# Biblbrox/ViT-Spectre-Experiments

Measured on AMD Instinct MI355X. Metric: images/sec training, Spectre-ViT-S CIFAR-100 bs512, higher is better.
Workload: dtype bf16; 1 GPU; Spectre-ViT-Small (E512 H16 F768 L4 P4 N65, 100 classes, dropout 0.001), fft mixer, train step fwd+CE+bwd+AdamW, bs 512/GPU; mixer=fft, global_batch=512, parallelism=dp1

## Files before the change

### vit-spectre-experiments_amd/csrc/spv_gemm.hip

```cpp
#define SPV_USES_SEED
#include "spv_common.h"
#include "spv_gemm_core.h"

#include <stdlib.h>

#include <algorithm>
#include <type_traits>

namespace {

constexpr int BM = GEMM_BM, BN = GEMM_BN;
constexpr int ROWB = 128 + 16;
constexpr int KBYTES = 128;

template <typename T> struct KT { static constexpr int BK = KBYTES / sizeof(T); static constexpr int CH = 16 / sizeof(T); };

template <typename TO> __device__ __forceinline__ void store_out(TO* p, float v);
template <> __device__ __forceinline__ void store_out<float>(float* p, float v) { *p = v; }
template <> __device__ __forceinline__ void store_out<bf16_t>(bf16_t* p, float v) { *p = f2bf(v); }
template <typename TO> __device__ __forceinline__ float load_out(const TO* p);
template <> __device__ __forceinline__ float load_out<float>(const float* p) { return *p; }
template <> __device__ __forceinline__ float load_out<bf16_t>(const bf16_t* p) { return bf2f(*p); }

__device__ __forceinline__ int xcd_remap(int id, int nwg) {
    int q = nwg >> 3, r = nwg & 7, x = id & 7;
    int base = (x < r) ? x * (q + 1) : r * (q + 1) + (x - r) * q;
    return base + (id >> 3);
}

__device__ __forceinline__ void tile_coords(int tile, int tiles_n, int tiles_mn, int& tm, int& tn) {
    constexpr int GM = 8;
    if (tiles_n <= 8) { tm = tile / tiles_n; tn = tile % tiles_n; return; }
    const int tiles_m = tiles_mn / tiles_n;
    const int per_group = GM * tiles_n;
    const int grp = tile / per_group, in = tile % per_group;
    const int m_first = grp * GM;
    const int gm = min(GM, tiles_m - m_first);
    tm = m_first + in % gm;
    tn = in / gm;
}

template <typename TO>
__device__ __forceinline__ void store_acc_tile(f32x16 (*acc)[2], unsigned char* smem, const float* __restrict__ bias,
                                               TO* __restrict__ C, float* __restrict__ ws, int M, int N, int ldc, int accumulate,
                                               int m0, int n0, int split, int rg, int gs, int roff,
                                               const float* __restrict__ bias2d, const void* __restrict__ bc = nullptr,
                                               int bc_pw = 0, int bc_bf = 0, int wrow = -1, int wcol = -1, float drop_p = 0.0f,
                                               uint64_t drop_seed = 0) {
    const int lane = threadIdx.x & 63, wave = threadIdx.x >> 6;
    const int fh = lane >> 5;
    if (wrow < 0) wrow = (wave >> 1) * 64;
    if (wcol < 0) wcol = (wave & 1) * 64;
    float* stage = reinterpret_cast<float*>(smem + wave * 9216);
    constexpr int SLD = 68;
    const bool vec_c = ((size_t)ldc * sizeof(TO)) % 16 == 0 && ((reinterpret_cast<uintptr_t>(C) | reinterpret_cast<uintptr_t>(bias)) & 15) == 0;
    const bool vec_ws = (N & 3) == 0;
    const uint64_t seed_live = drop_p > 0.0f ? live_seed(drop_seed) : 0;
#pragma unroll
    for (int i = 0; i < 2; ++i) {
        __syncthreads();
#pragma unroll
        for (int j = 0; j < 2; ++j)
#pragma unroll
            for (int r = 0; r < 16; ++r)
                stage[((r & 3) + 8 * (r >> 2) + 4 * fh) * SLD + j * 32 + (lane & 31)] = acc[i][j][r];
        __syncthreads();
#pragma unroll
        for (int t = 0; t < 4; ++t) {
            const int qd = lane + 64 * t;
            const int lr = qd >> 3, c8 = qd & 7;
            const int row = m0 + wrow + i * 32 + lr;
            const int col0 = n0 + wcol + c8 * 8;
            if (row >= M || col0 >= N) continue;
            float v[8];
            {
                const float4 lo = *reinterpret_cast<const float4*>(stage + lr * SLD + c8 * 8);
                const float4 hi = *reinterpret_cast<const float4*>(stage + lr * SLD + c8 * 8 + 4);
                v[0] = lo.x; v[1] = lo.y; v[2] = lo.z; v[3] = lo.w; v[4] = hi.x; v[5] = hi.y; v[6] = hi.z; v[7] = hi.w;
            }
            const int nvalid = min(8, N - col0);
            if (ws != nullptr) {
                float* wp = ws + ((size_t)split * M + row) * N + col0;
                if (nvalid == 8 && vec_ws) {
                    *reinterpret_cast<float4*>(wp) = make_float4(v[0], v[1], v[2], v[3]);
                    *reinterpret_cast<float4*>(wp + 4) = make_float4(v[4], v[5], v[6], v[7]);
                } else {
                    for (int u = 0; u < nvalid; ++u) wp[u] = v[u];
                }
                continue;
            }
            int orow = row;
            const float* b2 = nullptr;
            if (rg > 0) {
                orow = (row / rg) * gs + roff + (row % rg);
                if (bias2d) b2 = bias2d + (size_t)(row % rg) * N + col0;
            }
            TO* cp = C + (size_t)orow * ldc + col0;
            if (bc != nullptr) {
                const float sc = 1.0f / (float)bc_pw;
                const int ldp = N / bc_pw;
                if ((bc_pw & 7) == 0) {
                    const size_t o = (size_t)row * ldp + col0 / bc_pw;
                    const float t = (bc_bf ? bf2f(static_cast<const bf16_t*>(bc)[o]) : static_cast<const float*>(bc)[o]) * sc;
#pragma unroll
                    for (int u = 0; u < 8; ++u) v[u] += t;
                } else {
#pragma unroll
                    for (int u = 0; u < 8; ++u) {
                        if (u < nvalid) {
                            const size_t o = (size_t)row * ldp + (col0 + u) / bc_pw;
                            v[u] += (bc_bf ? bf2f(static_cast<const bf16_t*>(bc)[o]) : static_cast<const float*>(bc)[o]) * sc;
                        }
                    }
                }
            }
            if (nvalid == 8 && vec_c) {
                if (bias != nullptr) {
                    const float4 b0 = *reinterpret_cast<const float4*>(bias + col0), b1 = *reinterpret_cast<const float4*>(bias + col0 + 4);
                    v[0] += b0.x; v[1] += b0.y; v[2] += b0.z; v[3] += b0.w; v[4] += b1.x; v[5] += b1.y; v[6] += b1.z; v[7] += b1.w;
                }
                if (b2 != nullptr) {
                    if (vec_ws && (reinterpret_cast<uintptr_t>(bias2d) & 15) == 0) {
                        const float4 p0 = *reinterpret_cast<const float4*>(b2), p1 = *reinterpret_cast<const float4*>(b2 + 4);
                        v[0] += p0.x; v[1] += p0.y; v[2] += p0.z; v[3] += p0.w; v[4] += p1.x; v[5] += p1.y; v[6] += p1.z; v[7] += p1.w;
                    } else {
#pragma unroll
                        for (int u = 0; u < 8; ++u) v[u] += b2[u];
                    }
                }
                if (drop_p > 0.0f) {
                    const size_t fi = (size_t)orow * ldc + col0;
                    const unsigned key = dropout_row_key(seed_live, (uint64_t)fi >> 12);
                    const unsigned c0 = (unsigned)(fi & 4095);
                    const float inv_keep = 1.0f / (1.0f - drop_p);
                    const unsigned key_next = c0 > 4088u ? dropout_row_key(seed_live, ((uint64_t)fi >> 12) + 1) : key;
#pragma unroll
                    for (int u = 0; u < 8; ++u) v[u] *= dropout_scale(c0 + u < 4096u ? key : key_next, (c0 + u) & 4095u, drop_p, inv_keep);
                }
                if constexpr (sizeof(TO) == 2) {
                    if (accumulate) {
                        const uint4 old = *reinterpret_cast<const uint4*>(cp);
                        v[0] += __uint_as_float(old.x << 16); v[1] += __uint_as_float(old.x & 0xffff0000u);
                        v[2] += __uint_as_float(old.y << 16); v[3] += __uint_as_float(old.y & 0xffff0000u);
                        v[4] += __uint_as_float(old.z << 16); v[5] += __uint_as_float(old.z & 0xffff0000u);
                        v[6] += __uint_as_float(old.w << 16); v[7] += __uint_as_float(old.w & 0xffff0000u);
                    }
                    uint4 o;
                    o.x = pack_bf16x2(v[0], v[1]);
                    o.y = pack_bf16x2(v[2], v[3]);
                    o.z = pack_bf16x2(v[4], v[5]);
                    o.w = pack_bf16x2(v[6], v[7]);
                    *reinterpret_cast<uint4*>(cp) = o;
                } else {
                    float4* c4 = reinterpret_cast<float4*>(cp);
                    if (accumulate) {
                        const float4 o0 = c4[0], o1 = c4[1];
                        v[0] += o0.x; v[1] += o0.y; v[2] += o0.z; v[3] += o0.w; v[4] += o1.x; v[5] += o1.y; v[6] += o1.z; v[7] += o1.w;
                    }
                    c4[0] = make_float4(v[0], v[1], v[2], v[3]);
                    c4[1] = make_float4(v[4], v[5], v[6], v[7]);
                }
            } else {
                for (int u = 0; u < nvalid; ++u) {
                    float x = v[u];
                    if (bias != nullptr) x += bias[col0 + u];
                    if (b2 != nullptr) x += b2[u];
                    if (drop_p > 0.0f) {
                        const size_t fi = (size_t)orow * ldc + col0 + u;
                        x *= dropout_scale(dropout_row_key(seed_live, (uint64_t)fi >> 12), (unsigned)(fi & 4095), drop_p, 1.0f / (1.0f - drop_p));
                    }
                    if (accumulate) x += load_out<TO>(cp + u);
                    store_out<TO>(cp + u, x);
                }
            }
        }
    }
}

template <typename T, typename TO>
__global__ __launch_bounds__(256) void gemm_nt_kernel(const T* __restrict__ A, const T* __restrict__ B,
                                                      const float* __restrict__ bias, TO* __restrict__ C,
                                                      float* __restrict__ ws, int M, int N, int K, int lda,
                                                      int ldb, int ldc, int k_per_split, int accumulate,
                                                      int tiles_n, int tiles_mn, int nsplit, int rg, int gs, int roff,
                                                      const float* __restrict__ bias2d, const void* __restrict__ bc, int bc_pw,
                                                      int bc_bf, float drop_p, uint64_t drop_seed) {
    constexpr int BK = KT<T>::BK;
    constexpr int CH = KT<T>::CH;
    __shared__ __attribute__((aligned(16))) unsigned char smem[2 * BM * ROWB];
    unsigned char* sA = smem;
    unsigned char* sB = smem + BM * ROWB;

    const int tid = threadIdx.x;
    const int lane = tid & 63;
    const int wave = tid >> 6;
    const int wm = wave >> 1, wn = wave & 1;

    const int lin = xcd_remap(blockIdx.x, tiles_mn * nsplit);
    const int split = lin / tiles_mn;
    const int tile = lin % tiles_mn;
    int tm, tn;
    tile_coords(tile, tiles_n, tiles_mn, tm, tn);
// ... 901 lines not shown
            if (left == 3) step_noload(t + 1, a2, b2);
        }
        multiply(((nfull - 1) & 1) * WBUF, no{}, 0, a0, b0);
        __syncthreads();
    }
    if (krem > 0) {
        load_partial(kbeg + nfull * TBK, a0, b0);
        store_part(0, a0, b0, -1);
        __syncthreads();
        multiply(0, no{}, 0, a0, b0);
        __syncthreads();
    }
    store_acc_tile<TO>(acc, tw_smem, nullptr, C, ws, M, N, ldc, accumulate, m0, n0, split, 0, 0, 0, nullptr, nullptr, 0, 0, wm * 64, wn * 64);
}

constexpr int TW_SMEM_DB = 2 * (TBK * TWROWA + TBK * TROWB);
template <typename TO>
__global__ __launch_bounds__(512) void gemm_tn_wide_kernel(const bf16_t* __restrict__ A, const bf16_t* __restrict__ B, TO* __restrict__ C,
                                                           float* __restrict__ ws, int M, int N, int K, int lda, int ldb, int ldc,
                                                           int k_per_split, int accumulate, int tiles_n, int tiles_mn, int nsplit) {
    const int lin = xcd_remap(blockIdx.x, tiles_mn * nsplit);
    tn_wide_body<TO>(A, B, C, ws, M, N, K, lda, ldb, ldc, k_per_split, accumulate, tiles_n, lin % tiles_mn, lin / tiles_mn);
}

constexpr int TTM = GEMM_TTM;
constexpr int TTK = GEMM_TTK;
constexpr int TTROWA = TTM * 2 + 64;
constexpr int TT_SMEM = 2 * (TTK * TTROWA + TTK * TROWB);
template <typename TO>
__global__ __launch_bounds__(512) void gemm_tn_tall_kernel(const bf16_t* __restrict__ A, const bf16_t* __restrict__ B, TO* __restrict__ C,
                                                           float* __restrict__ ws, int M, int N, int K, int lda, int ldb, int ldc,
                                                           int k_per_split, int accumulate, int tiles_n, int tiles_mn, int nsplit) {
    extern __shared__ __attribute__((aligned(16))) unsigned char tt_smem[];
    constexpr int WBUF = TTK * TTROWA + TTK * TROWB;
    unsigned char* sA = tt_smem;
    unsigned char* sB = tt_smem + TTK * TTROWA;
    const int lin = xcd_remap(blockIdx.x, tiles_mn * nsplit);
    const int tile = lin % tiles_mn, split = lin / tiles_mn;
    const int tid = threadIdx.x, lane = tid & 63, wave = tid >> 6;
    const int wm = wave >> 1, wn = wave & 1;
    const int m0 = (tile / tiles_n) * TTM, n0 = (tile % tiles_n) * BN;
    const int kbeg = split * k_per_split;
    const int kend = min(K, kbeg + k_per_split);
    const int arow = tid >> 6, ach = tid & 63, brow = tid >> 4, bch = tid & 15;
    typedef tn_u32x4 RegA[4];
    RegA a0, a1, a2;
    tn_u32x4 b0, b1, b2;
    uint32_t aoff[4];
#pragma unroll
    for (int i = 0; i < 4; ++i) aoff[i] = (uint32_t)(((size_t)(arow + 8 * i) * lda + ach * 8) * 2);
    const uint32_t boff = (uint32_t)(((size_t)brow * ldb + bch * 8) * 2);
    const int nfull = (kend - kbeg) / TTK, krem = (kend - kbeg) % TTK;
    auto load_full = [&](int t, RegA& ra, tn_u32x4& rb) __attribute__((always_inline)) {
        const int k0 = kbeg + min(t, nfull - 1) * TTK;
        const unsigned char* ab = reinterpret_cast<const unsigned char*>(A + (size_t)k0 * lda + m0);
        const unsigned char* bb = reinterpret_cast<const unsigned char*>(B + (size_t)k0 * ldb + n0);
#pragma unroll
        for (int i = 0; i < 4; ++i) ra[i] = *reinterpret_cast<const tn_u32x4*>(ab + aoff[i]);
        rb = *reinterpret_cast<const tn_u32x4*>(bb + boff);
    };
    auto load_partial = [&](int k0, RegA& ra, tn_u32x4& rb) __attribute__((always_inline)) {
#pragma unroll
        for (int i = 0; i < 4; ++i) {
            const int k = k0 + arow + 8 * i;
            ra[i] = k < kend ? *reinterpret_cast<const tn_u32x4*>(A + (size_t)k * lda + m0 + ach * 8) : tn_u32x4{0u, 0u, 0u, 0u};
        }
        const int k = k0 + brow;
        rb = k < kend ? *reinterpret_cast<const tn_u32x4*>(B + (size_t)k * ldb + n0 + bch * 8) : tn_u32x4{0u, 0u, 0u, 0u};
    };
    auto store_part = [&](int buf, const RegA& ra, const tn_u32x4& rb, int ks) __attribute__((always_inline)) {
#pragma unroll
        for (int i = 0; i < 4; ++i)
            if (ks < 0 || ks == (i >= 3 ? 1 : 0)) *reinterpret_cast<tn_u32x4*>(sA + buf + (arow + 8 * i) * TTROWA + ach * 16) = ra[i];
        if (ks < 0 || ks == 1) *reinterpret_cast<tn_u32x4*>(sB + buf + brow * TROWB + bch * 16) = rb;
    };
    f32x16 acc[4][2];
#pragma unroll
    for (int i = 0; i < 4; ++i)
#pragma unroll
        for (int j = 0; j < 2; ++j)
#pragma unroll
            for (int r = 0; r < 16; ++r) acc[i][j][r] = 0.0f;
    const int g = lane >> 4, li = lane & 15, q = li >> 2, pp = li & 3;
    const unsigned char* fa0 = sA + (8 * (g >> 1) + q) * TTROWA + (16 * (g & 1) + 4 * pp) * 2 + (wm * 128) * 2;
    const unsigned char* fb0 = sB + (8 * (g >> 1) + q) * TROWB + (16 * (g & 1) + 4 * pp) * 2 + (wn * 64) * 2;
    using lds_ptr = s16x4 __attribute__((address_space(3)))*;
    auto fragA = [&](const unsigned char* p) __attribute__((always_inline)) {
        const s16x4 lo = __builtin_amdgcn_ds_read_tr16_b64_v4i16((lds_ptr)(p));
        const s16x4 hi = __builtin_amdgcn_ds_read_tr16_b64_v4i16((lds_ptr)(p + 4 * TTROWA));
        typedef __attribute__((ext_vector_type(8))) short s16x8;
        const s16x8 v = {lo[0], lo[1], lo[2], lo[3], hi[0], hi[1], hi[2], hi[3]};
        return __builtin_bit_cast(bf16x8, v);
    };
    auto multiply = [&](int cur, auto store_tag, int nxt, const RegA& ra, const tn_u32x4& rb) __attribute__((always_inline)) {
        constexpr bool STORE = decltype(store_tag)::value;
#pragma unroll
        for (int ks = 0; ks < TTK / 16; ++ks) {
            bf16x8 a[4], b[2];
#pragma unroll
            for (int f = 0; f < 4; ++f) a[f] = fragA(fa0 + cur + ks * 16 * TTROWA + f * 64);
#pragma unroll
            for (int f = 0; f < 2; ++f) b[f] = tr_frag(fb0 + cur + ks * 16 * TROWB + f * 64);
            if constexpr (STORE) store_part(nxt, ra, rb, ks);
#pragma unroll
            for (int i = 0; i < 4; ++i)
#pragma unroll
                for (int j = 0; j < 2; ++j)
                    acc[i][j] = __builtin_amdgcn_mfma_f32_32x32x16_bf16(a[i], b[j], acc[i][j], 0, 0, 0);
        }
    };
    using yes = std::true_type;
    using no = std::false_type;
    if (nfull > 0) {
        load_full(0, a0, b0);
        load_full(1, a1, b1);
        load_full(2, a2, b2);
        store_part(0, a0, b0, -1);
        load_full(3, a0, b0);
        __syncthreads();
        auto step = [&](int t, RegA& ra, tn_u32x4& rb) __attribute__((always_inline)) {
            multiply((t & 1) * WBUF, yes{}, ((t + 1) & 1) * WBUF, ra, rb);
            load_full(t + 4, ra, rb);
            __syncthreads();
        };
        auto step_noload = [&](int t, const RegA& ra, const tn_u32x4& rb) __attribute__((always_inline)) {
            multiply((t & 1) * WBUF, yes{}, ((t + 1) & 1) * WBUF, ra, rb);
            __syncthreads();
        };
        int t = 0;
        for (; t + 4 <= nfull; t += 3) {
            step(t, a1, b1);
            step(t + 1, a2, b2);
            step(t + 2, a0, b0);
        }
        const int left = nfull - t;
        if (left >= 2) {
            step_noload(t, a1, b1);
            if (left == 3) step_noload(t + 1, a2, b2);
        }
        multiply(((nfull - 1) & 1) * WBUF, no{}, 0, a0, b0);
        __syncthreads();
    }
    if (krem > 0) {
        load_partial(kbeg + nfull * TTK, a0, b0);
        store_part(0, a0, b0, -1);
        __syncthreads();
        multiply(0, no{}, 0, a0, b0);
        __syncthreads();
    }
    store_acc_tile<TO>(&acc[0], tt_smem, nullptr, C, ws, M, N, ldc, accumulate, m0, n0, split, 0, 0, 0, nullptr, nullptr, 0, 0, wm * 128, wn * 64);
    store_acc_tile<TO>(&acc[2], tt_smem, nullptr, C, ws, M, N, ldc, accumulate, m0, n0, split, 0, 0, 0, nullptr, nullptr, 0, 0, wm * 128 + 64, wn * 64);
}

__global__ __launch_bounds__(512) void gemm_tn_batch_wide_kernel(TnBatch tb, float* __restrict__ ws, int K, int k_per_split, int nsplit) {
    const TnWork w = tn_batch_work(tb, ws, K, k_per_split, nsplit);
    if (w.j < 0) return;
    const TnBatch::P& q = tb.p[w.j];
    tn_wide_body<float>(q.A, q.B, q.C, w.ws, q.M, q.N, w.K, q.lda, q.ldb, q.ldc, w.k_per_split, 0, q.tiles_n, w.tile, w.split);
}

template <typename TO>
__device__ __forceinline__ void splitk_reduce_body(const float* __restrict__ ws, const float* __restrict__ bias, TO* __restrict__ C, int M, int N,
                                                   int ldc, int splits, int accumulate, size_t bid, size_t nblocks, int tid, int nthreads) {
    const size_t total = (size_t)M * N;
    if ((N & 3) == 0) {
        const size_t quads = total >> 2;
        for (size_t qd = bid * nthreads + tid; qd < quads; qd += nblocks * nthreads) {
            const size_t e = qd << 2;
            const int row = (int)(e / N), col = (int)(e % N);
            float4 v = make_float4(0.0f, 0.0f, 0.0f, 0.0f);
            int sidx = 0;
            for (; sidx + 4 <= splits; sidx += 4) {
                const float4 a0 = *reinterpret_cast<const float4*>(ws + (size_t)(sidx + 0) * total + e);
                const float4 a1 = *reinterpret_cast<const float4*>(ws + (size_t)(sidx + 1) * total + e);
                const float4 a2 = *reinterpret_cast<const float4*>(ws + (size_t)(sidx + 2) * total + e);
                const float4 a3 = *reinterpret_cast<const float4*>(ws + (size_t)(sidx + 3) * total + e);
                v.x = (((v.x + a0.x) + a1.x) + a2.x) + a3.x;
                v.y = (((v.y + a0.y) + a1.y) + a2.y) + a3.y;
                v.z = (((v.z + a0.z) + a1.z) + a2.z) + a3.z;
                v.w = (((v.w + a0.w) + a1.w) + a2.w) + a3.w;
            }
            for (; sidx < splits; ++sidx) {
                const float4 a0 = *reinterpret_cast<const float4*>(ws + (size_t)sidx * total + e);
                v.x += a0.x; v.y += a0.y; v.z += a0.z; v.w += a0.w;
            }
            float o[4] = {v.x, v.y, v.z, v.w};
            TO* cp = C + (size_t)row * ldc + col;
#pragma unroll
            for (int u = 0; u < 4; ++u) {
                if (bias) o[u] += bias[col + u];
                if (accumulate) o[u] += load_out<TO>(cp + u);
                store_out<TO>(cp + u, o[u]);
            }
        }
        return;
    }
    for (size_t e = bid * nthreads + tid; e < total; e += nblocks * nthreads) {
        const int row = (int)(e / N), col = (int)(e % N);
        float v = 0.0f;
        for (int s = 0; s < splits; ++s) v += ws[(size_t)s * total + e];
        if (bias) v += bias[col];
        TO* cp = C + (size_t)row * ldc + col;
        if (accumulate) v += load_out<TO>(cp);
        store_out<TO>(cp, v);
    }
}

template <typename TO>
__global__ __launch_bounds__(256) void splitk_reduce_kernel(const float* __restrict__ ws, const float* __restrict__ bias,
                                                            TO* __restrict__ C, int M, int N, int ldc, int splits,
                                                            int accumulate) {
    splitk_reduce_body<TO>(ws, bias, C, M, N, ldc, splits, accumulate, blockIdx.x, gridDim.x, threadIdx.x, 256);
}

constexpr int FJ_MAX = GEMM_FJ_MAX;
static_assert(GEMM_FOLD_THREADS == FOLD_COLS * FOLD_ROWS, "spv_gemm_core.h sizes the batched reduce by the fold workgroup");
struct FoldJobs {
    int njobs;
    int first_block[FJ_MAX + 1];
    FoldJob job[FJ_MAX];
};
__device__ __forceinline__ void fold_jobs_block(const FoldJobs& fj, int bid, int tid) {
    int j = 0;
    while (j + 1 < fj.njobs && bid >= fj.first_block[j + 1]) ++j;
    fold_partials_block(fj.job[j], bid - fj.first_block[j], tid);
}
constexpr int FOLD_NARROW = 4;
__global__ __launch_bounds__(FOLD_COLS * FOLD_ROWS / FOLD_NARROW) void fold_multi_kernel(FoldJobs fj) {
    int j = 0;
    while (j + 1 < fj.njobs && (int)blockIdx.x >= fj.first_block[j + 1]) ++j;
    fold_partials_block<FOLD_NARROW>(fj.job[j], blockIdx.x - fj.first_block[j], threadIdx.x);
}

template <typename TO>
__global__ __launch_bounds__(FOLD_COLS * FOLD_ROWS) void splitk_reduce_fold_kernel(const float* __restrict__ ws, TO* __restrict__ C, int M, int N,
                                                                                   int ldc, int splits, int accumulate, int reduce_blocks,
                                                                                   FoldJobs fj) {
    const int fold_blocks = fj.first_block[fj.njobs];
    if ((int)blockIdx.x < fold_blocks)
        fold_jobs_block(fj, (int)blockIdx.x, threadIdx.x);
    else if (threadIdx.x < 256)
        splitk_reduce_body<TO>(ws, nullptr, C, M, N, ldc, splits, accumulate, blockIdx.x - fold_blocks, reduce_blocks, threadIdx.x, 256);
}

__global__ __launch_bounds__(FOLD_COLS * FOLD_ROWS) void splitk_reduce_batch_kernel(TnBatch tb, const float* __restrict__ ws, int splits,
                                                                                    int reduce_blocks, FoldJobs fj) {
    const int fold_blocks = fj.njobs > 0 ? fj.first_block[fj.njobs] : 0;
    if ((int)blockIdx.x < fold_blocks) {
        fold_jobs_block(fj, (int)blockIdx.x, threadIdx.x);
    } else {
        const int b = (int)blockIdx.x - fold_blocks;
        const int j = b / reduce_blocks;
        const TnBatch::P& q = tb.p[j];
        splitk_reduce_body<float>(ws + tb.ws_off[j], nullptr, q.C, q.M, q.N, q.ldc, splits, 0, b % reduce_blocks, reduce_blocks, threadIdx.x,
                                  FOLD_COLS * FOLD_ROWS);
    }
}

static thread_local float t_drop_p = 0.0f;
static thread_local uint64_t t_drop_seed = 0;

inline int ptr_lo(const void* p) { return p == nullptr ? -1 : (int)(reinterpret_cast<uintptr_t>(p) & 15); }

template <typename T, typename TO>
int launch_gemm(const GemmNtPlan& pl, const void* A, const void* B, const float* bias, void* C, int M, int N, int K, int lda, int ldb,
                int ldc, int accumulate, void* workspace, hipStream_t st, int rg, int gs, int roff, const float* bias2d, const void* bc,
                int bc_pw, int bc_bf) {
    const int tiles_m = cdiv(M, BM), tiles_n = cdiv(N, BN);
    const int splits = pl.splits, k_per_split = pl.k_per_split;
    float* ws = splits > 1 ? static_cast<float*>(workspace) : nullptr;
    const dim3 grid(pl.grid);
    switch (pl.kernel) {
    case GEMM_NT_ROWS:
        if constexpr (sizeof(T) == 2) {
            hipLaunchKernelGGL((gemm_nt_rows_kernel<TO>), grid, dim3(256), 0, st, static_cast<const bf16_t*>(A), static_cast<const bf16_t*>(B), bias,
                               static_cast<TO*>(C), M, N, K, lda, ldb, ldc, accumulate, cdiv(N, 32));
            SPV_LAUNCH_CHECK("spv_gemm_nt(rows)");
            SPV_COUNT_PATH(SPV_PATH_GEMM_ROWS);
            return 0;
        }
        return spv_set_error("spv_gemm_nt: the rows kernel takes bf16 operands");
    case GEMM_NT_STRIP:
        if constexpr (sizeof(T) == 2 && sizeof(TO) == 2) {
            const int nwg = pl.grid;
#define SPV_STRIP(MBV, EPIV)                                                                                                \
    hipLaunchKernelGGL((gemm_nt_strip_kernel<MBV, EPIV>), dim3(nwg), dim3(512), 0, st, static_cast<const bf16_t*>(A),       \
                       static_cast<const bf16_t*>(B), bias, static_cast<bf16_t*>(C), M, K, lda, ldb, ldc, pl.nstrips, pl.base, pl.rem, nwg, \
                       static_cast<const bf16_t*>(bc), bc_pw, bc ? N / bc_pw : 0)
#define SPV_STRIP_MB(EPIV)                  \
    do {                                    \
        if (pl.mb == 4) SPV_STRIP(4, EPIV); \
        else if (pl.mb == 3) SPV_STRIP(3, EPIV); \
        else SPV_STRIP(2, EPIV);            \
    } while (0)
            SPV_COUNT_PATH(pl.epi >= 2 ? SPV_PATH_GEMM_STRIP_POOL : pl.epi == 1 ? SPV_PATH_GEMM_STRIP_ACC : SPV_PATH_GEMM_STRIP);
            switch (pl.epi) {
            case 3: SPV_STRIP_MB(3); break;
            case 2: SPV_STRIP_MB(2); break;
            case 1: SPV_STRIP_MB(1); break;
            default: SPV_STRIP_MB(0); break;
            }
#undef SPV_STRIP_MB
#undef SPV_STRIP
            SPV_LAUNCH_CHECK("spv_gemm_nt(strip)");
            return 0;
        }
        return spv_set_error("spv_gemm_nt: the strip kernel takes bf16 operands and a bf16 output");
    case GEMM_NT_GLDS:
        if constexpr (sizeof(T) == 2) {
            hipLaunchKernelGGL((gemm_nt_glds_kernel<TO, 128, 2>), grid, dim3(256), 0, st, static_cast<const bf16_t*>(A),
                               static_cast<const bf16_t*>(B), bias, static_cast<TO*>(C), ws, M, N, K, lda, ldb, ldc, k_per_split,
// ... 124 lines not shown
static int gemm_tn_impl(const void* A, const void* B, void* C, int M, int N, int K, int lda, int ldb, int ldc, int out_dtype,
                        int accumulate, int splits, void* workspace, void* stream, const spv_fold_job* folds, int nfolds) {
    FoldJobs fj{};
    const int fold_blocks = fold_blocks_of(folds, nfolds, fj);
    const GemmTnPlan pl = gemm_tn_plan(out_dtype, M, N, K, lda, ldb, ldc, ptr_lo(A), ptr_lo(B), splits, ptr_lo(workspace), fold_blocks);
    SPV_CHECK(pl.kernel != GEMM_TN_REFUSE_EMPTY, "spv_gemm_tn: empty problem M=%d N=%d K=%d", M, N, K);
    SPV_CHECK(pl.kernel != GEMM_TN_REFUSE_DTYPE, "spv_gemm_tn: bad out_dtype %d", out_dtype);
    SPV_CHECK(pl.kernel != GEMM_TN_REFUSE_CHUNK, "spv_gemm_tn: M=%d N=%d lda=%d ldb=%d must be multiples of 8 (bf16, 16-byte chunks)", M, N, lda, ldb);
    SPV_CHECK(pl.kernel != GEMM_TN_REFUSE_ALIGN, "spv_gemm_tn: A/B must be 16-byte aligned");
    SPV_CHECK(pl.kernel != GEMM_TN_REFUSE_LD, "spv_gemm_tn: leading dimension too small");
    SPV_CHECK(pl.kernel != GEMM_TN_REFUSE_WORKSPACE, "spv_gemm_tn: split-K needs a 16-byte aligned workspace (splits=%d)", splits);
    SPV_CHECK(pl.kernel != GEMM_TN_REFUSE_FOLDS, "spv_gemm_tn_fold: 0..%d fold jobs, each with partials, parts > 0, nsum 1..5, n > 0 and out[0]", FJ_MAX);
    SPV_COUNT_PATH(SPV_PATH_GEMM_TN);
    hipStream_t st = static_cast<hipStream_t>(stream);
    const int tiles_m = cdiv(M, BM), tiles_n = cdiv(N, BN);
    splits = pl.splits;
    const int k_per_split = pl.k_per_split;
    float* ws = splits > 1 ? static_cast<float*>(workspace) : nullptr;
    const dim3 grid(pl.grid);
    const bool bf = out_dtype == SPV_BF16;
    switch (pl.kernel) {
    case GEMM_TN_TALL:
        if (bf) {
            (void)hipFuncSetAttribute(reinterpret_cast<const void*>(&gemm_tn_tall_kernel<bf16_t>), hipFuncAttributeMaxDynamicSharedMemorySize, TT_SMEM);
            hipLaunchKernelGGL((gemm_tn_tall_kernel<bf16_t>), grid, dim3(512), TT_SMEM, st, (const bf16_t*)A, (const bf16_t*)B, (bf16_t*)C, ws, M, N, K, lda, ldb,
                               ldc, k_per_split, accumulate, tiles_n, tiles_n, splits);
        } else {
            (void)hipFuncSetAttribute(reinterpret_cast<const void*>(&gemm_tn_tall_kernel<float>), hipFuncAttributeMaxDynamicSharedMemorySize, TT_SMEM);
            hipLaunchKernelGGL((gemm_tn_tall_kernel<float>), grid, dim3(512), TT_SMEM, st, (const bf16_t*)A, (const bf16_t*)B, (float*)C, ws, M, N, K, lda, ldb,
                               ldc, k_per_split, accumulate, tiles_n, tiles_n, splits);
        }
        SPV_LAUNCH_CHECK("spv_gemm_tn(tall)");
        break;
    case GEMM_TN_WIDE: {
        const int wt = (M / TWM) * tiles_n;
#define SPV_TNW(TOV)                                                                                                                      \
    do {                                                                                                                                  \
        (void)hipFuncSetAttribute(reinterpret_cast<const void*>(&gemm_tn_wide_kernel<TOV>), hipFuncAttributeMaxDynamicSharedMemorySize, TW_SMEM_DB); \
        hipLaunchKernelGGL((gemm_tn_wide_kernel<TOV>), grid, dim3(512), TW_SMEM_DB, st, (const bf16_t*)A, (const bf16_t*)B, (TOV*)C,     \
                           ws, M, N, K, lda, ldb, ldc, k_per_split, accumulate, tiles_n, wt, splits);                                     \
    } while (0)
        if (bf) SPV_TNW(bf16_t);
        else SPV_TNW(float);
#undef SPV_TNW
        SPV_LAUNCH_CHECK("spv_gemm_tn(wide)");
        SPV_COUNT_PATH(SPV_PATH_GEMM_TN_WIDE);
        break;
    }
    case GEMM_TN_TILE1:
    case GEMM_TN_TILE3:
#define SPV_TN(TOV, DV)                                                                                                     \
    hipLaunchKernelGGL((gemm_tn_kernel<TOV, DV>), grid, dim3(256), 0, st, (const bf16_t*)A, (const bf16_t*)B, (TOV*)C, ws, M, N, K, \
                       lda, ldb, ldc, k_per_split, accumulate, tiles_n, tiles_m * tiles_n, splits)
        if (bf) {
            if (pl.kernel == GEMM_TN_TILE1) SPV_TN(bf16_t, 1); else SPV_TN(bf16_t, 3);
        } else {
            if (pl.kernel == GEMM_TN_TILE1) SPV_TN(float, 1); else SPV_TN(float, 3);
        }
#undef SPV_TN
        SPV_LAUNCH_CHECK("spv_gemm_tn");
        break;
    default:
        return spv_set_error("spv_gemm_tn: no kernel for plan %d", (int)pl.kernel);
    }
    switch (pl.reduce) {
    case GEMM_TN_REDUCE_FOLDS:
        if (bf)
            hipLaunchKernelGGL((splitk_reduce_fold_kernel<bf16_t>), dim3(pl.reduce_blocks + fold_blocks), dim3(FOLD_COLS * FOLD_ROWS), 0, st, ws, (bf16_t*)C, M, N,
                               ldc, splits, accumulate, pl.reduce_blocks, fj);
        else
            hipLaunchKernelGGL((splitk_reduce_fold_kernel<float>), dim3(pl.reduce_blocks + fold_blocks), dim3(FOLD_COLS * FOLD_ROWS), 0, st, ws, (float*)C, M, N,
                               ldc, splits, accumulate, pl.reduce_blocks, fj);
        SPV_LAUNCH_CHECK("spv_gemm_tn_fold(split-k reduce + fold)");
        break;
    case GEMM_TN_REDUCE_PLAIN:
        if (bf)
            hipLaunchKernelGGL((splitk_reduce_kernel<bf16_t>), dim3(pl.reduce_blocks), dim3(256), 0, st, ws, (const float*)nullptr, (bf16_t*)C, M, N,
                               ldc, splits, accumulate);
        else
            hipLaunchKernelGGL((splitk_reduce_kernel<float>), dim3(pl.reduce_blocks), dim3(256), 0, st, ws, (const float*)nullptr, (float*)C, M, N, ldc,
                               splits, accumulate);
        SPV_LAUNCH_CHECK("spv_gemm_tn(split-k reduce)");
        break;
    case GEMM_TN_FOLD_ALONE:
        hipLaunchKernelGGL(fold_multi_kernel, dim3(fold_blocks), dim3(FOLD_COLS * FOLD_ROWS / FOLD_NARROW), 0, st, fj);
        SPV_LAUNCH_CHECK("spv_gemm_tn_fold(fold)");
        break;
    case GEMM_TN_NO_REDUCE:
        break;
    }
    return 0;
}

extern "C" int spv_gemm_tn(const void* A, const void* B, void* C, int M, int N, int K, int lda, int ldb, int ldc, int out_dtype,
                           int accumulate, int splits, void* workspace, void* stream) {
    return gemm_tn_impl(A, B, C, M, N, K, lda, ldb, ldc, out_dtype, accumulate, splits, workspace, stream, nullptr, 0);
}

extern "C" int spv_gemm_tn_fold(const void* A, const void* B, void* C, int M, int N, int K, int lda, int ldb, int ldc, int out_dtype,
                                int accumulate, int splits, void* workspace, const spv_fold_job* folds, int nfolds, void* stream) {
    return gemm_tn_impl(A, B, C, M, N, K, lda, ldb, ldc, out_dtype, accumulate, splits, workspace, stream, folds, nfolds);
}

extern "C" int spv_fold_multi(const spv_fold_job* folds, int nfolds, void* stream) {
    SPV_CHECK(folds != nullptr && nfolds > 0, "spv_fold_multi: no jobs");
    hipStream_t st = static_cast<hipStream_t>(stream);
    for (int j0 = 0; j0 < nfolds; j0 += FJ_MAX) {
        FoldJobs fj{};
        int blocks = 0;
        SPV_CHECK(fill_fold_jobs(folds + j0, std::min(FJ_MAX, nfolds - j0), fj, blocks) == 0, "spv_fold_multi: bad fold job");
        hipLaunchKernelGGL(fold_multi_kernel, dim3(blocks), dim3(FOLD_COLS * FOLD_ROWS / FOLD_NARROW), 0, st, fj);
        SPV_LAUNCH_CHECK("spv_fold_multi");
    }
    return 0;
}

static int gemm_tn_batch_impl(const spv_tn_problem* probs, int nprob, int K, int splits, void* workspace, const spv_fold_job* folds,
                              int nfolds, void* stream, int parts) {
    FoldJobs fj{};
    const int fold_blocks = fold_blocks_of(folds, nfolds, fj);
    GemmTnBatchProblem qs[TNB_MAX];
    const bool listed = probs != nullptr && nprob >= 1 && nprob <= TNB_MAX;
    for (int i = 0; listed && i < nprob; ++i) {
        const spv_tn_problem& q = probs[i];
        qs[i] = {q.m, q.n, q.lda, q.ldb, q.ldc, q.k, ptr_lo(q.a), ptr_lo(q.b), q.a != nullptr && q.b != nullptr && q.c != nullptr};
    }
    const GemmTnBatchPlan pl = gemm_tn_batch_plan(listed ? qs : nullptr, nprob, K, splits, ptr_lo(workspace), fold_blocks);
    SPV_CHECK(pl.kernel != GEMM_TNB_REFUSE_COUNT, "spv_gemm_tn_batch: 1..%d problems", TNB_MAX);
    SPV_CHECK(pl.kernel != GEMM_TNB_REFUSE_CALL, "spv_gemm_tn_batch: K=%d splits=%d need a 16-byte aligned workspace", K, splits);
    SPV_CHECK(pl.kernel != GEMM_TNB_REFUSE_FOLDS, "spv_gemm_tn_batch: 0..%d fold jobs, each with partials, parts > 0, nsum 1..5, n > 0 and out[0]", FJ_MAX);
    SPV_CHECK(pl.kernel != GEMM_TNB_REFUSE_K, "spv_gemm_tn_batch: problem %d: k must be 0 (= K) or 1..K=%d", pl.bad, K);
    SPV_CHECK(pl.kernel != GEMM_TNB_REFUSE_NO_LONG, "spv_gemm_tn_batch: no problem reduces over the call's K=%d rows", K);
    SPV_CHECK(pl.kernel != GEMM_TNB_REFUSE_EMPTY, "spv_gemm_tn_batch: empty problem %d", pl.bad);
    SPV_CHECK(pl.kernel != GEMM_TNB_REFUSE_SHAPE, "spv_gemm_tn_batch: problem %d: M, N, lda, ldb must be multiples of 8, leading dimensions >= extents", pl.bad);
    SPV_CHECK(pl.kernel != GEMM_TNB_REFUSE_ALIGN, "spv_gemm_tn_batch: problem %d: A/B must be 16-byte aligned", pl.bad);
    SPV_CHECK(pl.kernel != GEMM_TNB_REFUSE_SHORT_LDC, "spv_gemm_tn_batch: problem %d (short): ldc must be a multiple of 4", pl.bad);
    TnBatch tb{};
    tb.nprob = nprob;
    tb.nlong = pl.nlong;
    const bool wide = pl.kernel == GEMM_TNB_WIDE;
    for (int i = 0; i < nprob; ++i) {
        const spv_tn_problem& q = probs[pl.order[i]];
        tb.first_tile[i] = wide ? pl.wide_first_tile[i] : pl.first_tile[i];
        tb.ws_off[i] = pl.ws_off[i];
        tb.p[i] = {static_cast<const bf16_t*>(q.a), static_cast<const bf16_t*>(q.b), static_cast<float*>(q.c), q.m, q.n, q.lda, q.ldb, q.ldc, cdiv(q.n, BN),
                   i < pl.nlong ? K : q.k};
    }
    tb.first_tile[nprob] = wide ? pl.wide_first_tile[nprob] : pl.first_tile[nprob];
    hipStream_t st = static_cast<hipStream_t>(stream);
    if (parts & 1) {
        SPV_COUNT_PATH(SPV_PATH_GEMM_TN);
        SPV_COUNT_PATH(SPV_PATH_GEMM_TN_BATCH);
        if (wide) {
            (void)hipFuncSetAttribute(reinterpret_cast<const void*>(&gemm_tn_batch_wide_kernel), hipFuncAttributeMaxDynamicSharedMemorySize, TW_SMEM_DB);
            hipLaunchKernelGGL(gemm_tn_batch_wide_kernel, dim3(pl.grid), dim3(512), TW_SMEM_DB, st, tb, static_cast<float*>(workspace), K, pl.k_per_split, pl.splits);
            SPV_COUNT_PATH(SPV_PATH_GEMM_TN_WIDE);
        } else {
            hipLaunchKernelGGL(gemm_tn_batch_kernel<3>, dim3(pl.grid), dim3(256), 0, st, tb, static_cast<float*>(workspace), K, pl.k_per_split, pl.splits);
        }
        SPV_LAUNCH_CHECK("spv_gemm_tn_batch");
    }
    if (parts & 2) {
        hipLaunchKernelGGL(splitk_reduce_batch_kernel, dim3(fold_blocks + pl.nlong * pl.reduce_blocks), dim3(FOLD_COLS * FOLD_ROWS), 0, st, tb,
                           static_cast<const float*>(workspace), pl.splits, pl.reduce_blocks, fj);
        SPV_LAUNCH_CHECK("spv_gemm_tn_batch(split-k reduce + fold)");
    }
    return 0;
}

extern "C" int spv_gemm_tn_batch(const spv_tn_problem* probs, int nprob, int K, int splits, void* workspace, const spv_fold_job* folds,
                                 int nfolds, void* stream) {
    return gemm_tn_batch_impl(probs, nprob, K, splits, workspace, folds, nfolds, stream, 3);
}

extern "C" int spv_gemm_tn_batch_part(const spv_tn_problem* probs, int nprob, int K, int splits, void* workspace, const spv_fold_job* folds,
                                      int nfolds, int part, void* stream) {
    SPV_CHECK(part == 1 || part == 2, "spv_gemm_tn_batch_part: part must be 1 (the GEMM launch) or 2 (the reduce + fold launch), got %d", part);
    return gemm_tn_batch_impl(probs, nprob, K, splits, workspace, folds, nfolds, stream, part);
}
```

### vit-spectre-experiments_amd/csrc/spv_gemm_core.h

```cpp
#pragma once
#include <stddef.h>
#include <stdint.h>

constexpr int GEMM_BM = 128, GEMM_BN = 128;
constexpr int GEMM_GBK = 64;
constexpr int GEMM_TBK = 64;
constexpr int GEMM_TWM = 256;
constexpr int GEMM_TTM = 512, GEMM_TTK = 32;
constexpr int GEMM_TNB_MAX = 8;
constexpr int GEMM_FJ_MAX = 16;
constexpr int GEMM_FOLD_THREADS = 1024;
constexpr int GEMM_DT_F32 = 0, GEMM_DT_BF16 = 1;

inline int gemm_cdiv(int64_t a, int64_t b) { return (int)((a + b - 1) / b); }
inline int gemm_reduce_blocks(int M, int N, int threads) {
    const int64_t b = ((int64_t)M * N / ((N & 3) == 0 ? 4 : 1) + threads - 1) / threads;
    return (int)(b < 2048 ? b : 2048);
}

inline bool strip_plan(int M, int N, int K, int reserved_cus, int& MB, int& nstrips, int& groups, int& base, int& rem) {
    if (N <= 0 || N % 256 != 0 || N > 16384 || K % 128 != 0 || K < 128 || M < 8192) return false;
    nstrips = N / 256;
    const int nblk = gemm_cdiv(M, 32);
    groups = (256 - reserved_cus) / nstrips;
// ... 108 lines not shown
    return p;
}

enum GemmTnKernel : int {
    GEMM_TN_REFUSE_EMPTY = 0,
    GEMM_TN_REFUSE_DTYPE,
    GEMM_TN_REFUSE_CHUNK,
    GEMM_TN_REFUSE_ALIGN,
    GEMM_TN_REFUSE_LD,
    GEMM_TN_REFUSE_WORKSPACE,
    GEMM_TN_REFUSE_FOLDS,
    GEMM_TN_TALL,
    GEMM_TN_WIDE,
    GEMM_TN_TILE1,
    GEMM_TN_TILE3,
    GEMM_TN_KERNEL_COUNT
};
inline const char* gemm_tn_kernel_name(int k) {
    static const char* const names[GEMM_TN_KERNEL_COUNT] = {"refuse_empty", "refuse_dtype", "refuse_chunk", "refuse_align", "refuse_ld", "refuse_workspace",
                                                            "refuse_folds", "tall", "wide", "tile1", "tile3"};
    return k >= 0 && k < GEMM_TN_KERNEL_COUNT ? names[k] : "?";
}
enum GemmTnReduce : int {
    GEMM_TN_NO_REDUCE = 0,
    GEMM_TN_REDUCE_PLAIN,
    GEMM_TN_REDUCE_FOLDS,
    GEMM_TN_FOLD_ALONE
};
struct GemmTnPlan {
    GemmTnKernel kernel;
    GemmTnReduce reduce;
    int splits, k_per_split;
    int grid;
    int reduce_blocks;
};
inline GemmTnPlan gemm_tn_plan(int out_dtype, int M, int N, int K, int lda, int ldb, int ldc, int a_lo, int b_lo, int splits, int ws_lo, int fold_blocks) {
    GemmTnPlan p{};
    auto refuse = [&](GemmTnKernel k) { p.kernel = k; return p; };
    if (!(M > 0 && N > 0 && K > 0)) return refuse(GEMM_TN_REFUSE_EMPTY);
    if (out_dtype != GEMM_DT_F32 && out_dtype != GEMM_DT_BF16) return refuse(GEMM_TN_REFUSE_DTYPE);
    if (!(M % 8 == 0 && N % 8 == 0 && lda % 8 == 0 && ldb % 8 == 0)) return refuse(GEMM_TN_REFUSE_CHUNK);
    if (!(a_lo == 0 && b_lo == 0)) return refuse(GEMM_TN_REFUSE_ALIGN);
    if (!(lda >= M && ldb >= N && ldc >= N)) return refuse(GEMM_TN_REFUSE_LD);
    if (!(splits >= 1 && (splits == 1 || ws_lo == 0))) return refuse(GEMM_TN_REFUSE_WORKSPACE);
    if (fold_blocks < 0) return refuse(GEMM_TN_REFUSE_FOLDS);
    const int tiles_m = gemm_cdiv(M, GEMM_BM), tiles_n = gemm_cdiv(N, GEMM_BN);
    p.splits = 1;
    p.k_per_split = K;
    if (splits > 1) {
        p.k_per_split = gemm_cdiv(gemm_cdiv(K, splits), GEMM_TBK) * GEMM_TBK;
        p.splits = gemm_cdiv(K, p.k_per_split);
    }
    constexpr int wide_min = 4;
    if (M == GEMM_TTM && N % GEMM_BN == 0 && N >= 8 * GEMM_BN && tiles_n * p.splits >= 192 && p.k_per_split >= 16 * GEMM_TTK) {
        p.kernel = GEMM_TN_TALL;
        p.grid = tiles_n * p.splits;
    } else if (p.splits >= wide_min && M % GEMM_TWM == 0 && N % GEMM_BN == 0 && (M / GEMM_TWM) * tiles_n * p.splits >= 128) {
        p.kernel = GEMM_TN_WIDE;
        p.grid = (M / GEMM_TWM) * tiles_n * p.splits;
    } else {
        p.kernel = N <= 64 ? GEMM_TN_TILE1 : GEMM_TN_TILE3;
        p.grid = tiles_m * tiles_n * p.splits;
    }
    p.reduce = p.splits > 1 ? (fold_blocks > 0 ? GEMM_TN_REDUCE_FOLDS : GEMM_TN_REDUCE_PLAIN) : (fold_blocks > 0 ? GEMM_TN_FOLD_ALONE : GEMM_TN_NO_REDUCE);
    p.reduce_blocks = p.splits > 1 ? gemm_reduce_blocks(M, N, 256) : 0;
    return p;
}

enum GemmTnBatchKernel : int {
    GEMM_TNB_REFUSE_COUNT = 0,
    GEMM_TNB_REFUSE_CALL,
    GEMM_TNB_REFUSE_FOLDS,
    GEMM_TNB_REFUSE_K,
    GEMM_TNB_REFUSE_NO_LONG,
    GEMM_TNB_REFUSE_EMPTY,
    GEMM_TNB_REFUSE_SHAPE,
    GEMM_TNB_REFUSE_ALIGN,
    GEMM_TNB_REFUSE_SHORT_LDC,
    GEMM_TNB_128,
    GEMM_TNB_WIDE,
    GEMM_TNB_KERNEL_COUNT
};
inline const char* gemm_tnb_kernel_name(int k) {
    static const char* const names[GEMM_TNB_KERNEL_COUNT] = {"refuse_count", "refuse_call", "refuse_folds", "refuse_k", "refuse_no_long", "refuse_empty",
                                                             "refuse_shape", "refuse_align", "refuse_short_ldc", "batch128", "batch_wide"};
    return k >= 0 && k < GEMM_TNB_KERNEL_COUNT ? names[k] : "?";
}
struct GemmTnBatchProblem {
    int m, n, lda, ldb, ldc, k;
    int a_lo, b_lo;
    int has_ptrs;
};
struct GemmTnBatchPlan {
    GemmTnBatchKernel kernel;
    int bad;
    int splits, k_per_split;
    int nlong;
    int order[GEMM_TNB_MAX];
    int first_tile[GEMM_TNB_MAX + 1];
    int wide_first_tile[GEMM_TNB_MAX + 1];
    long long ws_off[GEMM_TNB_MAX];
    int grid;
    int reduce_blocks;
};
inline GemmTnBatchPlan gemm_tn_batch_plan(const GemmTnBatchProblem* q, int nprob, int K, int splits, int ws_lo, int fold_blocks) {
    GemmTnBatchPlan p{};
    p.bad = -1;
    auto refuse = [&](GemmTnBatchKernel k, int which) { p.kernel = k; p.bad = which; return p; };
    if (!(q != nullptr && nprob >= 1 && nprob <= GEMM_TNB_MAX)) return refuse(GEMM_TNB_REFUSE_COUNT, -1);
    if (!(K > 0 && splits >= 1 && ws_lo == 0)) return refuse(GEMM_TNB_REFUSE_CALL, -1);
    if (fold_blocks < 0) return refuse(GEMM_TNB_REFUSE_FOLDS, -1);
    p.k_per_split = gemm_cdiv(gemm_cdiv(K, splits), GEMM_TBK) * GEMM_TBK;
    p.splits = gemm_cdiv(K, p.k_per_split);
    int no = 0;
    for (int i = 0; i < nprob; ++i) {
        if (!(q[i].k >= 0 && q[i].k <= K)) return refuse(GEMM_TNB_REFUSE_K, i);
        if (q[i].k == 0 || q[i].k == K) p.order[no++] = i;
    }
    p.nlong = no;
    for (int i = 0; i < nprob; ++i)
        if (!(q[i].k == 0 || q[i].k == K)) p.order[no++] = i;
    if (p.nlong < 1) return refuse(GEMM_TNB_REFUSE_NO_LONG, -1);
    int tiles = 0, wt = 0, long_tiles = 0, wlong = 0;
    long long off = 0;
    p.reduce_blocks = 1;
    bool wide = p.k_per_split >= 8 * GEMM_TBK;
    for (int i = 0; i < nprob; ++i) {
        const GemmTnBatchProblem& r = q[p.order[i]];
        if (!(r.has_ptrs && r.m > 0 && r.n > 0)) return refuse(GEMM_TNB_REFUSE_EMPTY, p.order[i]);
        if (!(r.m % 8 == 0 && r.n % 8 == 0 && r.lda % 8 == 0 && r.ldb % 8 == 0 && r.lda >= r.m && r.ldb >= r.n && r.ldc >= r.n))
            return refuse(GEMM_TNB_REFUSE_SHAPE, p.order[i]);
        if (!(r.a_lo == 0 && r.b_lo == 0)) return refuse(GEMM_TNB_REFUSE_ALIGN, p.order[i]);
        if (!(i < p.nlong || r.ldc % 4 == 0)) return refuse(GEMM_TNB_REFUSE_SHORT_LDC, p.order[i]);
        wide = wide && r.m % GEMM_TWM == 0 && r.n % GEMM_BN == 0 && (r.k == 0 || r.k >= GEMM_TBK);
        p.first_tile[i] = tiles;
        p.wide_first_tile[i] = wt;
        p.ws_off[i] = off;
        tiles += gemm_cdiv(r.m, GEMM_BM) * gemm_cdiv(r.n, GEMM_BN);
        wt += (r.m / GEMM_TWM) * gemm_cdiv(r.n, GEMM_BN);
        if (i < p.nlong) {
            long_tiles = tiles;
            wlong = wt;
            off += (long long)p.splits * r.m * r.n;
            const int rb = gemm_reduce_blocks(r.m, r.n, GEMM_FOLD_THREADS);
            if (rb > p.reduce_blocks) p.reduce_blocks = rb;
        }
    }
    p.first_tile[nprob] = tiles;
    p.wide_first_tile[nprob] = wt;
    p.kernel = wide ? GEMM_TNB_WIDE : GEMM_TNB_128;
    p.grid = wide ? wlong * p.splits + ((wt - wlong + 7) & ~7) : long_tiles * p.splits + ((tiles - long_tiles + 7) & ~7);
    return p;
}
```

Baseline: 326,800 images/sec.

## Make batched TN wide GEMM persistent with XCD-aware work scheduling and epilogue overlap

Replaces the one-tile-per-workgroup launch of the batched transposed-A wide GEMM with a persistent kernel sized to the CU count. Each workgroup walks a static work list in which short problems come first and split-K long items are grouped per XCD for L2 locality. The global loads for the next item are issued before the current tile's accumulator store, so the epilogue overlaps with the next prologue. The cost is extra register pressure, more complex index math and a one-time device attribute query on the host.

```diff
diff --git a/vit-spectre-experiments_amd/csrc/spv_gemm.hip b/vit-spectre-experiments_amd/csrc/spv_gemm.hip
--- a/vit-spectre-experiments_amd/csrc/spv_gemm.hip
+++ b/vit-spectre-experiments_amd/csrc/spv_gemm.hip
@@ -46,8 +46,9 @@
                                                int m0, int n0, int split, int rg, int gs, int roff,
                                                const float* __restrict__ bias2d, const void* __restrict__ bc = nullptr,
                                                int bc_pw = 0, int bc_bf = 0, int wrow = -1, int wcol = -1, float drop_p = 0.0f,
-                                               uint64_t drop_seed = 0) {
-    const int lane = threadIdx.x & 63, wave = threadIdx.x >> 6;
+                                               uint64_t drop_seed = 0, int tid = -1) {
+    if (tid < 0) tid = threadIdx.x;
+    const int lane = tid & 63, wave = tid >> 6;
     const int fh = lane >> 5;
     if (wrow < 0) wrow = (wave >> 1) * 64;
     if (wcol < 0) wcol = (wave & 1) * 64;
@@ -1255,11 +1256,184 @@
     store_acc_tile<TO>(&acc[2], tt_smem, nullptr, C, ws, M, N, ldc, accumulate, m0, n0, split, 0, 0, 0, nullptr, nullptr, 0, 0, wm * 128 + 64, wn * 64);
 }
 
-__global__ __launch_bounds__(512) void gemm_tn_batch_wide_kernel(TnBatch tb, float* __restrict__ ws, int K, int k_per_split, int nsplit) {
-    const TnWork w = tn_batch_work(tb, ws, K, k_per_split, nsplit);
-    if (w.j < 0) return;
-    const TnBatch::P& q = tb.p[w.j];
-    tn_wide_body<float>(q.A, q.B, q.C, w.ws, q.M, q.N, w.K, q.lda, q.ldb, q.ldc, w.k_per_split, 0, q.tiles_n, w.tile, w.split);
+struct TnItem {
+    const bf16_t* A;
+    const bf16_t* B;
+    float* C;
+    float* ws;
+    int M, N, lda, ldb, ldc, m0, n0, split, kbeg, kend;
+};
+__device__ __forceinline__ TnItem tn_batch_item(const TnBatch& tb, float* ws, int K, int k_per_split, int nshort, int id) {
+    const int long_tiles = tb.first_tile[tb.nlong];
+    int split = 0, t;
+    if (id < nshort) {
+        t = long_tiles + id;
+    } else {
+        split = (id - nshort) / long_tiles;
+        t = (id - nshort) % long_tiles;
+    }
+    int j = 0;
+    while (j + 1 < tb.nprob && t >= tb.first_tile[j + 1]) ++j;
+    const TnBatch::P& q = tb.p[j];
+    const bool is_long = j < tb.nlong;
+    const int tile = t - tb.first_tile[j];
+    const int kk = is_long ? K : q.K, kps = is_long ? k_per_split : q.K;
+    return {q.A, q.B, q.C, is_long ? ws + tb.ws_off[j] : nullptr, q.M, q.N, q.lda, q.ldb, q.ldc, (tile / q.tiles_n) * TWM, (tile % q.tiles_n) * BN,
+            split, split * kps, min(kk, split * kps + kps)};
+}
+__global__ __launch_bounds__(512) void gemm_tn_batch_wide_kernel(TnBatch tb, GemmTnbWorkPlan wp, float* __restrict__ ws, int K, int k_per_split) {
+    extern __shared__ __attribute__((aligned(16))) unsigned char tw_smem[];
+    unsigned char* sA = tw_smem;
+    unsigned char* sB = tw_smem + TBK * TWROWA;
+    const int tid = threadIdx.x, lane = tid & 63, wave = tid >> 6;
+    const int wm = wave >> 1, wn = wave & 1;
+    const int arow = tid >> 5, ach = tid & 31, brow = tid >> 4, bch = tid & 15;
+    typedef tn_u32x4 RegA[4];
+    typedef tn_u32x4 RegB[2];
+    RegA a0, a1, a2;
+    RegB b0, b1, b2;
+    uint32_t aoff[4], boff[2];
+    TnItem it;
+    int nfull = 0;
+    auto open_item = [&](int id) __attribute__((always_inline)) {
+        it = tn_batch_item(tb, ws, K, k_per_split, wp.nshort, id);
+        nfull = (it.kend - it.kbeg) / TBK;
+        int otid = tid;
+        asm volatile("" : "+v"(otid));
+#pragma unroll
+        for (int i = 0; i < 4; ++i) aoff[i] = (uint32_t)(((size_t)((otid >> 5) + 16 * i) * it.lda + (otid & 31) * 8) * 2);
+#pragma unroll
+        for (int i = 0; i < 2; ++i) boff[i] = (uint32_t)(((size_t)((otid >> 4) + 32 * i) * it.ldb + (otid & 15) * 8) * 2);
+    };
+    auto load_full = [&](int t, RegA& ra, RegB& rb) __attribute__((always_inline)) {
+        const int k0 = it.kbeg + min(t, nfull - 1) * TBK;
+        const unsigned char* ab = reinterpret_cast<const unsigned char*>(it.A + (size_t)k0 * it.lda + it.m0);
+        const unsigned char* bb = reinterpret_cast<const unsigned char*>(it.B + (size_t)k0 * it.ldb + it.n0);
+#pragma unroll
+        for (int i = 0; i < 4; ++i) ra[i] = *reinterpret_cast<const tn_u32x4*>(ab + aoff[i]);
+#pragma unroll
+        for (int i = 0; i < 2; ++i) rb[i] = *reinterpret_cast<const tn_u32x4*>(bb + boff[i]);
+    };
+    auto load_partial = [&](int k0, RegA& ra, RegB& rb) __attribute__((always_inline)) {
+#pragma unroll
+        for (int i = 0; i < 4; ++i) {
+            const int k = k0 + arow + 16 * i;
+            ra[i] = k < it.kend ? *reinterpret_cast<const tn_u32x4*>(it.A + (size_t)k * it.lda + it.m0 + ach * 8) : tn_u32x4{0u, 0u, 0u, 0u};
+        }
+#pragma unroll
+        for (int i = 0; i < 2; ++i) {
+            const int k = k0 + brow + 32 * i;
+            rb[i] = k < it.kend ? *reinterpret_cast<const tn_u32x4*>(it.B + (size_t)k * it.ldb + it.n0 + bch * 8) : tn_u32x4{0u, 0u, 0u, 0u};
+        }
+    };
+    auto store_part = [&](int boff_lds, const RegA& ra, const RegB& rb, int ks) __attribute__((always_inline)) {
+#pragma unroll
+        for (int i = 0; i < 4; ++i)
+            if (ks < 0 || ks == (i >> 1)) *reinterpret_cast<tn_u32x4*>(sA + boff_lds + (arow + 16 * i) * TWROWA + ach * 16) = ra[i];
+#pragma unroll
+        for (int i = 0; i < 2; ++i)
+            if (ks < 0 || ks == 2 + i) *reinterpret_cast<tn_u32x4*>(sB + boff_lds + (brow + 32 * i) * TROWB + bch * 16) = rb[i];
+    };
+    f32x16 acc[2][2];
+    const int g = lane >> 4, li = lane & 15, q = li >> 2, pp = li & 3;
+    const unsigned char* fa0 = sA + (8 * (g >> 1) + q) * TWROWA + (16 * (g & 1) + 4 * pp) * 2 + (wm * 64) * 2;
+    const unsigned char* fb0 = sB + (8 * (g >> 1) + q) * TROWB + (16 * (g & 1) + 4 * pp) * 2 + (wn * 64) * 2;
+    using lds_ptr = s16x4 __attribute__((address_space(3)))*;
+    auto fragA = [&](const unsigned char* p) __attribute__((always_inline)) {
+        const s16x4 lo = __builtin_amdgcn_ds_read_tr16_b64_v4i16((lds_ptr)(p));
+        const s16x4 hi = __builtin_amdgcn_ds_read_tr16_b64_v4i16((lds_ptr)(p + 4 * TWROWA));
+        typedef __attribute__((ext_vector_type(8))) short s16x8;
+        const s16x8 v = {lo[0], lo[1], lo[2], lo[3], hi[0], hi[1], hi[2], hi[3]};
+        return __builtin_bit_cast(bf16x8, v);
+    };
+    auto multiply = [&](int cur, auto store_tag, int nxt, const RegA& ra, const RegB& rb) __attribute__((always_inline)) {
+        constexpr bool STORE = decltype(store_tag)::value;
+#pragma unroll
+        for (int ks = 0; ks < TBK / 16; ++ks) {
+            bf16x8 a[2], b[2];
+#pragma unroll
+            for (int f = 0; f < 2; ++f) {
+                a[f] = fragA(fa0 + cur + ks * 16 * TWROWA + f * 64);
+                b[f] = tr_frag(fb0 + cur + ks * 16 * TROWB + f * 64);
+            }
+            if constexpr (STORE) store_part(nxt, ra, rb, ks);
+#pragma unroll
+            for (int i = 0; i < 2; ++i)
+#pragma unroll
+                for (int j = 0; j < 2; ++j)
+                    acc[i][j] = __builtin_amdgcn_mfma_f32_32x32x16_bf16(a[i], b[j], acc[i][j], 0, 0, 0);
+        }
+    };
+    using yes = std::true_type;
+    using no = std::false_type;
+    constexpr int WBUF = TBK * TWROWA + TBK * TROWB;
+
+    int r = 0;
+    int id = gemm_tnb_work_item(wp, blockIdx.x, 0);
+    open_item(id);
+    if (nfull > 0) {
+        load_full(0, a0, b0);
+        load_full(1, a1, b1);
+        load_full(2, a2, b2);
+    }
+    while (true) {
+#pragma unroll
+        for (int i = 0; i < 2; ++i)
+#pragma unroll
+            for (int j = 0; j < 2; ++j)
+#pragma unroll
+                for (int e = 0; e < 16; ++e) acc[i][j][e] = 0.0f;
+        if (nfull > 0) {
+            store_part(0, a0, b0, -1);
+            load_full(3, a0, b0);
+            __syncthreads();
+            auto step = [&](int t, RegA& ra, RegB& rb) __attribute__((always_inline)) {
+                multiply((t & 1) * WBUF, yes{}, ((t + 1) & 1) * WBUF, ra, rb);
+                load_full(t + 4, ra, rb);
+                __syncthreads();
+            };
+            auto step_noload = [&](int t, const RegA& ra, const RegB& rb) __attribute__((always_inline)) {
+                multiply((t & 1) * WBUF, yes{}, ((t + 1) & 1) * WBUF, ra, rb);
+                __syncthreads();
+            };
+            int t = 0;
+            for (; t + 4 <= nfull; t += 3) {
+                step(t, a1, b1);
+                step(t + 1, a2, b2);
+                step(t + 2, a0, b0);
+            }
+            const int left = nfull - t;
+            if (left >= 2) {
+                step_noload(t, a1, b1);
+                if (left == 3) step_noload(t + 1, a2, b2);
+            }
+            multiply(((nfull - 1) & 1) * WBUF, no{}, 0, a0, b0);
+            __syncthreads();
+        }
+        if ((it.kend - it.kbeg) % TBK > 0) {
+            load_partial(it.kbeg + nfull * TBK, a0, b0);
+            store_part(0, a0, b0, -1);
+            __syncthreads();
+            multiply(0, no{}, 0, a0, b0);
+            __syncthreads();
+        }
+        const TnItem done = it;
+        id = gemm_tnb_work_item(wp, blockIdx.x, ++r);
+        if (id >= 0) {
+            open_item(id);
+            if (nfull > 0) {
+                load_full(0, a0, b0);
+                load_full(1, a1, b1);
+                load_full(2, a2, b2);
+            }
+        }
+        int etid = tid;
+        asm volatile("" : "+v"(etid));
+        store_acc_tile<float>(acc, tw_smem, nullptr, done.C, done.ws, done.M, done.N, done.ldc, 0, done.m0, done.n0, done.split, 0, 0, 0, nullptr, nullptr, 0,
+                              0, (etid >> 7) * 64, ((etid >> 6) & 1) * 64, 0.0f, 0, etid);
+        if (id < 0) break;
+        __syncthreads();
+    }
 }
 
 template <typename TO>
@@ -1690,8 +1864,17 @@
         SPV_COUNT_PATH(SPV_PATH_GEMM_TN);
         SPV_COUNT_PATH(SPV_PATH_GEMM_TN_BATCH);
         if (wide) {
+            static int cus = 0;
+            if (cus == 0) {
+                int dev = 0, v = 0;
+                SPV_CHECK(hipGetDevice(&dev) == hipSuccess && hipDeviceGetAttribute(&v, hipDeviceAttributeMultiprocessorCount, dev) == hipSuccess && v > 0,
+                          "spv_gemm_tn_batch: no device to size the grid for");
+                cus = v;
+            }
+            const int long_tiles = pl.wide_first_tile[pl.nlong];
+            const GemmTnbWorkPlan wp = gemm_tnb_work_plan(pl.wide_first_tile[nprob] - long_tiles, long_tiles * pl.splits, std::max(1, cus - g_reserved_cus));
             (void)hipFuncSetAttribute(reinterpret_cast<const void*>(&gemm_tn_batch_wide_kernel), hipFuncAttributeMaxDynamicSharedMemorySize, TW_SMEM_DB);
-            hipLaunchKernelGGL(gemm_tn_batch_wide_kernel, dim3(pl.grid), dim3(512), TW_SMEM_DB, st, tb, static_cast<float*>(workspace), K, pl.k_per_split, pl.splits);
+            hipLaunchKernelGGL(gemm_tn_batch_wide_kernel, dim3(wp.wgs), dim3(512), TW_SMEM_DB, st, tb, wp, static_cast<float*>(workspace), K, pl.k_per_split);
             SPV_COUNT_PATH(SPV_PATH_GEMM_TN_WIDE);
         } else {
             hipLaunchKernelGGL(gemm_tn_batch_kernel<3>, dim3(pl.grid), dim3(256), 0, st, tb, static_cast<float*>(workspace), K, pl.k_per_split, pl.splits);
diff --git a/vit-spectre-experiments_amd/csrc/spv_gemm_core.h b/vit-spectre-experiments_amd/csrc/spv_gemm_core.h
--- a/vit-spectre-experiments_amd/csrc/spv_gemm_core.h
+++ b/vit-spectre-experiments_amd/csrc/spv_gemm_core.h
@@ -284,3 +284,39 @@
     p.grid = wide ? wlong * p.splits + ((wt - wlong + 7) & ~7) : long_tiles * p.splits + ((tiles - long_tiles + 7) & ~7);
     return p;
 }
+
+#if defined(__HIPCC__)
+#define GEMM_HD __host__ __device__
+#else
+#define GEMM_HD
+#endif
+struct GemmTnbWorkPlan {
+    int nshort, nlong, total;
+    int wgs;
+    int xcd_base[8];
+    int xcd_short[8];
+};
+inline GemmTnbWorkPlan gemm_tnb_work_plan(int short_tiles, int long_items, int cus) {
+    GemmTnbWorkPlan p{};
+    p.nshort = short_tiles;
+    p.nlong = long_items;
+    p.total = short_tiles + long_items;
+    p.wgs = p.total < cus ? p.total : cus;
+    if (p.wgs < 1) p.wgs = 1;
+    int base = 0;
+    for (int x = 0; x < 8; ++x) {
+        const int gx = x < p.wgs ? (p.wgs - x + 7) / 8 : 0;
+        auto upto = [&](int n) { return (n / p.wgs) * gx + (n % p.wgs > x ? (n % p.wgs - x + 7) / 8 : 0); };
+        p.xcd_short[x] = upto(p.nshort);
+        p.xcd_base[x] = base;
+        base += upto(p.total) - p.xcd_short[x];
+    }
+    return p;
+}
+GEMM_HD inline int gemm_tnb_work_item(const GemmTnbWorkPlan& p, int w, int r) {
+    const long long i = (long long)w + (long long)r * p.wgs;
+    if (i >= p.total) return -1;
+    if (i < p.nshort) return (int)i;
+    const int x = w & 7;
+    return p.nshort + p.xcd_base[x] + r * ((p.wgs - x + 7) / 8) + (w >> 3) - p.xcd_short[x];
+}
```

After: 329,200 images/sec (median of 6 runs). Within noise of the previous version (+0.7%).
